# asonnino/hotstuff

Measured on NVIDIA H100. Metric: Ed25519 verifies/s, higher is better.
Workload: dtype u32

## Files before the change

hotstuff_b200/csrc/hs_engine.cu:

```cuda
#include <cuda_runtime.h>
#include <algorithm>
#include <array>
#include <atomic>
#include <condition_variable>
#include <cstdint>
#include <cstdio>
#include <cstdlib>
#include <cstring>
#include <deque>
#include <initializer_list>
#include <list>
#include <memory>
#include <mutex>
#include <new>
#include <optional>
#include <random>
#include <string>
#include <string_view>
#include <thread>
#include <unordered_map>
#include <vector>

#include "../../include/hs_crypto.h"
#include "hs_args.h"
#include "hs_selftest_vectors.h"
#include "verify_core.cuh"

#define HS_THREADS 128
#define HS_FINISH_GROUP 16
#define HS_NO_KEY 0xffffffffu
#define HS_LEARN_MAX 8192u
#define HS_LEARN_PER_CALL 1024u
#define HS_CACHE_RESET_MIN_CALLS 64u

struct in_layout {
  const uint8_t *sig;
  size_t sig_stride;
  const uint8_t *pk;
  size_t pk_stride;
  const uint32_t *vidx;
  const uint8_t *msg;
  size_t msg_stride;
  const uint32_t *midx;
  const uint64_t *off;
  uint64_t fixed_len;
  int aos128;
};

__device__ __forceinline__ void load32(uint32_t (&w)[8], const uint8_t *p) {
  const uint32_t *s = reinterpret_cast<const uint32_t *>(p);
#pragma unroll
  for (int i = 0; i < 8; i++) w[i] = __ldg(s + i);
}
__device__ __forceinline__ void unpack8(uint32_t (&w)[8], uint4 lo, uint4 hi) {
  w[0] = lo.x; w[1] = lo.y; w[2] = lo.z; w[3] = lo.w;
  w[4] = hi.x; w[5] = hi.y; w[6] = hi.z; w[7] = hi.w;
}
__device__ __forceinline__ void store_digest32(uint32_t *dst, const uint32_t *h) {
  uint4 *d = reinterpret_cast<uint4 *>(dst);
  d[0] = make_uint4(h[0], h[1], h[2], h[3]);
  d[1] = make_uint4(h[4], h[5], h[6], h[7]);
}
// ... 59 lines not shown
    h = (h + 1) & T.mask;
  }
  return HS_NO_KEY;
}
__global__ void __launch_bounds__(256) k_key_lookup(in_layout L, size_t n, key_table T, uint32_t *__restrict__ out_vidx,
                                                    uint32_t *__restrict__ miss_list, uint32_t *__restrict__ miss_count) {
  const size_t i = (size_t)blockIdx.x * 256 + threadIdx.x;
  if (i >= n) return;
  uint32_t k[8];
  load32(k, L.pk + i * L.pk_stride);
  uint32_t pos;
  const uint32_t found = key_probe<false>(T, k, pos);
  out_vidx[i] = found;
  if (found == HS_NO_KEY) miss_list[atomicAdd(miss_count, 1u)] = (uint32_t)i;
}

__global__ void __launch_bounds__(256) k_gather_keys(in_layout L, size_t n, const uint32_t *__restrict__ miss_list,
                                                     const uint32_t *__restrict__ miss_count, uint32_t max_keys, uint8_t *__restrict__ out_keys,
                                                     uint32_t *__restrict__ out_n) {
  const size_t t = (size_t)blockIdx.x * 256 + threadIdx.x;
  const size_t avail = miss_count ? (size_t)*miss_count : n;
  const size_t take = avail < max_keys ? avail : max_keys;
  if (t == 0) *out_n = (uint32_t)take;
  if (t >= take) return;
  const size_t i = miss_count ? miss_list[t] : t;
  uint32_t k[8];
  load32(k, L.pk + i * L.pk_stride);
  uint32_t *dst = reinterpret_cast<uint32_t *>(out_keys + t * 32);
#pragma unroll
  for (int j = 0; j < 8; j++) dst[j] = k[j];
}

struct main_out {
  fe *xyz;
  uint8_t *meta;
  int side_pass;
};
struct committee_tables {
  const uint8_t *pks;
  const uint8_t *key_flags;
  uint32_t n_keys;
  const ge_niels *atables;
  size_t table_entries;
};

template <bool COMMITTEE>
#ifndef HS_MAIN_MINBLOCKS
#define HS_MAIN_MINBLOCKS 4
#endif
#ifndef HS_GENERIC_MINBLOCKS
#define HS_GENERIC_MINBLOCKS 3
#endif
__global__ void __launch_bounds__(HS_THREADS, COMMITTEE ? HS_MAIN_MINBLOCKS : HS_GENERIC_MINBLOCKS) k_verify_main(in_layout L, size_t n_arg, const uint32_t *__restrict__ n_ptr,
                                                             const uint32_t *__restrict__ index_list, const ge_niels *__restrict__ btable,
                                                             committee_tables C, main_out O, const comb_params cp) {
  __shared__ __align__(16) unsigned char smem_raw[HS_MAX_DIGITS * HS_THREADS * 4];
  static_assert(sizeof(smem_raw) >= (HS_THREADS / 32) * 256 * sizeof(uint4), "staging does not fit");
  uint4(*stage)[256] = reinterpret_cast<uint4(*)[256]>(smem_raw);
  int32_t *digits = reinterpret_cast<int32_t *>(smem_raw) + threadIdx.x;
  const size_t n = n_ptr ? (size_t)*n_ptr : n_arg;
  for (size_t base = (size_t)blockIdx.x * blockDim.x; base < n; base += (size_t)gridDim.x * blockDim.x) {
  const size_t t = base + threadIdx.x;
  const size_t warp_first = t & ~(size_t)31;
  const bool active = t < n;
  size_t i = active ? t : n - 1;
  uint32_t R[8], S[8], A[8], h[16];
  uint32_t v = 0;
// ... 27 lines not shown
    if (len == 32 && ((reinterpret_cast<uintptr_t>(m) & 3u) == 0)) {
      uint32_t M[8];
      load32(M, m);
      sha512_ram32(h, R, A, M);
    } else {
      uint64_t pre[8];
#pragma unroll
      for (int j = 0; j < 4; j++) {
        pre[j] = be64_from_le32(R[2 * j], R[2 * j + 1]);
        pre[4 + j] = be64_from_le32(A[2 * j], A[2 * j + 1]);
      }
      sha512_prefix_msg(h, pre, 8, m, len);
    }
  }
  ge_ext acc;
  uint32_t meta;
  if (COMMITTEE) {
    meta = verify_committee_main(acc, R, S, h, btable, C.atables + (size_t)v * C.table_entries, have_key ? C.key_flags[v] : 0u, digits,
                                 HS_THREADS, cp);
    if (!have_key) {
      if (O.side_pass) continue;
      meta = 0;
    }
  } else {
    ge_cached tab[9];
    meta = verify_generic_main(acc, R, S, A, h, btable, tab, digits, HS_THREADS, cp);
  }
  if (!active) continue;
  if (!(meta & HS_META_PARSE_OK)) {
    fe_set0(acc.X);
    fe_set1(acc.Y);
    fe_set1(acc.Z);
  }
  uint4 *dst = reinterpret_cast<uint4 *>(O.xyz + i * 3);
  dst[0] = make_uint4(acc.X.v[0], acc.X.v[1], acc.X.v[2], acc.X.v[3]);
  dst[1] = make_uint4(acc.X.v[4], acc.X.v[5], acc.X.v[6], acc.X.v[7]);
  dst[2] = make_uint4(acc.Y.v[0], acc.Y.v[1], acc.Y.v[2], acc.Y.v[3]);
  dst[3] = make_uint4(acc.Y.v[4], acc.Y.v[5], acc.Y.v[6], acc.Y.v[7]);
  dst[4] = make_uint4(acc.Z.v[0], acc.Z.v[1], acc.Z.v[2], acc.Z.v[3]);
  dst[5] = make_uint4(acc.Z.v[4], acc.Z.v[5], acc.Z.v[6], acc.Z.v[7]);
  O.meta[i] = (uint8_t)meta;
  }
}

struct small_rec {
  uint8_t sig[64];
  uint8_t msg[32];
  uint32_t vidx;
  uint32_t req;
  uint32_t req_n;
  uint32_t pad[5];
};
static_assert(sizeof(small_rec) == 128, "small_rec is 128 bytes");
#define HS_SMALL_MAX 64
__device__ __forceinline__ void fe_shfl_down(fe &r, const fe &a, int delta) {
#pragma unroll
  for (int i = 0; i < 8; i++) r.v[i] = __shfl_down_sync(0xffffffffu, a.v[i], delta);
}

#define HS_SIG_WAYS 4
struct sig_entry {
  uint32_t w[32];
  uint32_t seq;
  uint32_t flags;
  uint32_t pad[2];
};
static_assert(sizeof(sig_entry) == 144, "sig_entry is 144 bytes");
struct sig_bucket {
  sig_entry e[HS_SIG_WAYS];
  uint32_t rr;
  uint32_t pad[3];
};
#define HS_SIG_CTRS 4
// ... 450 lines not shown
  int n;
  int my_rank;
  uint32_t epoch;
  size_t total_words;
  size_t word_offset;
};
#define HS_PEER_FLAGS(P) ((P).total_words * 2)
#define HS_PEER_CTRL(P) ((P).total_words * 2 + HS_MAX_PEERS)
__device__ __forceinline__ void peer_signal_and_wait(const peer_route &P) {
  const int p = threadIdx.x;
  if (p >= P.n) return;
  uint32_t *own = P.buf[P.my_rank];
  __threadfence_system();
  asm volatile("st.release.sys.global.u32 [%0], %1;" ::"l"(P.buf[p] + HS_PEER_FLAGS(P) + P.my_rank), "r"(P.epoch) : "memory");
  uint32_t v = 0;
  bool ok = false;
  for (long long spin = 0; spin < (1ll << 24); spin++) {
    asm volatile("ld.acquire.sys.global.u32 %0, [%1];" : "=r"(v) : "l"(own + HS_PEER_FLAGS(P) + p) : "memory");
    if ((int32_t)(v - P.epoch) >= 0) {
      ok = true;
      break;
    }
    __nanosleep(200);
  }
  if (!ok) {
    own[HS_PEER_CTRL(P)] = 1;
    const size_t per = P.total_words / P.n;
    uint32_t *w = own + (P.epoch & 1u) * P.total_words + (size_t)p * per;
    for (size_t k = 0; k < per; k++) w[k] = 0;
  }
}
__global__ void k_peer_sync_only(const peer_route P) { peer_signal_and_wait(P); }

__device__ __forceinline__ void fe_load_global(fe &r, const fe *p) {
  const uint4 *s = reinterpret_cast<const uint4 *>(p);
  unpack8(r.v, s[0], s[1]);
}
__host__ __device__ inline uint32_t mode_flag(uint32_t mode) { return mode == HS_MODE_BATCH_EQ ? HS_F_EQ : HS_F_STRICT; }
template <class Verdict>
__device__ __forceinline__ void verify_finish_body(const in_layout &L, size_t n, const fe *__restrict__ xyz, const uint8_t *__restrict__ meta,
                                                   Verdict verdict, uint32_t *__restrict__ bitmap, const peer_route &P, const int group) {
  __shared__ fe tot[HS_THREADS];
  const size_t t = (size_t)blockIdx.x * HS_THREADS + threadIdx.x;
  const size_t first = t * (size_t)group;
  const int cnt = (first < n) ? (int)((n - first < (size_t)group) ? (n - first) : group) : 0;
  fe prod[HS_FINISH_GROUP];
  fe run;
  fe_set1(run);
#pragma unroll 1
  for (int c = 0; c < cnt; c++) {
    fe Z;
    fe_load_global(Z, xyz + (first + c) * 3 + 2);
    if (fe_is_zero(Z)) fe_set1(Z);
    fe_mul(run, run, Z);
    prod[c] = run;
  }
  tot[threadIdx.x] = run;
  __syncthreads();
  block_invert4(tot);
  __syncthreads();
  uint32_t bits = 0;
  if (cnt) {
    fe u = tot[threadIdx.x];
#pragma unroll 1
    for (int c = cnt - 1; c >= 0; c--) {
      const size_t i = first + c;
      fe X, Y, Z, zinv;
      fe_load_global(X, xyz + i * 3 + 0);
      fe_load_global(Y, xyz + i * 3 + 1);
      fe_load_global(Z, xyz + i * 3 + 2);
      const uint32_t zero_z = fe_is_zero(Z);
      if (zero_z) fe_set1(Z);
      if (c > 0) fe_mul(zinv, u, prod[c - 1]);
      else zinv = u;
      fe_mul(u, u, Z);
      uint32_t R[8];
      load32(R, L.sig + i * L.sig_stride);
      uint32_t m = meta[i];
      if (zero_z) m &= ~HS_META_PARSE_OK;
      const uint32_t fl = verify_flags_from(X, Y, zinv, R, m);
      const uint32_t ok = verdict(i, fl);
      if (ok) bits |= 1u << c;
    }
  }
  const int lanes_per_word = 32 / group;
  uint32_t word = bits << (group * (threadIdx.x & (lanes_per_word - 1)));
  for (int m = 1; m < lanes_per_word; m <<= 1) word |= __shfl_xor_sync(0xffffffffu, word, m);
  if ((threadIdx.x & (lanes_per_word - 1)) == 0 && first < n) {
    const size_t widx = t / lanes_per_word;
    if (P.n == 0) {
      bitmap[widx] = word;
    } else {
      const size_t at = (P.epoch & 1u) * P.total_words + P.word_offset + widx;
#pragma unroll 1
      for (int p = 0; p < P.n; p++) P.buf[p][at] = word;
    }
  }
  if (P.n) {
    __shared__ int is_last;
    __threadfence_system();
    __syncthreads();
    if (threadIdx.x == 0) is_last = atomicAdd(P.buf[P.my_rank] + HS_PEER_CTRL(P) + 1, 1u) == gridDim.x - 1;
    __syncthreads();
    if (is_last) {
      peer_signal_and_wait(P);
      __syncthreads();
      if (threadIdx.x == 0) P.buf[P.my_rank][HS_PEER_CTRL(P) + 1] = 0;
    }
  }
}
__global__ void __launch_bounds__(HS_THREADS) k_verify_finish(in_layout L, size_t n, const fe *__restrict__ xyz, const uint8_t *__restrict__ meta,
                                                               uint32_t mode, uint32_t *__restrict__ bitmap, const peer_route P, const int group) {
  verify_finish_body(L, n, xyz, meta, [&](size_t, uint32_t fl) { return fl & mode_flag(mode); }, bitmap, P, group);
}
__global__ void __launch_bounds__(HS_THREADS) k_verify_finish_modes(in_layout L, size_t n, const fe *__restrict__ xyz, const uint8_t *__restrict__ meta,
                                                                     const uint8_t *__restrict__ item_mode, uint32_t *__restrict__ bitmap, const peer_route P,
                                                                     const int group) {
  verify_finish_body(L, n, xyz, meta, [&](size_t i, uint32_t fl) { return fl & mode_flag(item_mode[i]); }, bitmap, P, group);
}

#define HS_BUILD_BLOCK 64
__global__ void __launch_bounds__(HS_THREADS) k_build_comb(const uint8_t *__restrict__ encs, size_t n_points, int negate, int W, int n_windows,
                                                            ge_niels *tables, uint8_t *key_flags) {
  const int entries = 1 << (W - 1);
  const int blocks_per_window = entries / HS_BUILD_BLOCK;
  const size_t t = (size_t)blockIdx.x * HS_THREADS + threadIdx.x;
  const size_t per_point = (size_t)n_windows * blocks_per_window;
  const size_t p = t / per_point;
  if (p >= n_points) return;
  const int w = (int)((t % per_point) / blocks_per_window);
  const int b = (int)(t % blocks_per_window);
  ge_ext P;
  if (encs) {
    uint32_t e[8];
    load32(e, encs + p * 32);
    uint32_t ok = ge_decompress(P, e);
    uint32_t small = ge_enc_is_small_order(e);
    if (w == 0 && b == 0 && key_flags) key_flags[p] = (uint8_t)((ok & 1u) | (small << 1));
    if (!ok) ge_identity(P);
  } else {
    ge_basepoint(P);
  }
  if (negate) {
    ge_ext Q;
    ge_neg(Q, P);
    P = Q;
  }
  fe prod[HS_BUILD_BLOCK];
  comb_build_block(tables + p * ((size_t)n_windows * comb_window_stride(W)), P, W, w, b * HS_BUILD_BLOCK, HS_BUILD_BLOCK, prod);
}
// ... 643 lines not shown
  if (!c->cache_enabled || c->explicit_committee || c->learn_pending || !L.pk) return HS_OK;
  if (!c->learn.keys) {
    learn_bufs B;
    HS_CUDA(c, alloc(B.keys, (size_t)HS_LEARN_MAX * 32));
    HS_CUDA(c, alloc(B.n, 4));
    HS_CUDA(c, alloc(B.h_keys, (size_t)HS_LEARN_MAX * 32));
    HS_CUDA(c, alloc(B.h_n, 4));
    HS_CUDA(c, alloc(B.h_miss_total, 4));
    HS_CUDA(c, create(B.ev));
    HS_CUDA(c, create(B.ev_tables));
    c->learn = std::move(B);
  }
  learn_bufs &B = c->learn;
  c->learn_records = n;
  if (c->cache_full) {
    if (!have_lookup) return HS_OK;
    HS_CUDA(c, cudaMemcpyAsync(B.h_miss_total, c->d_miss_count, 4, cudaMemcpyDeviceToHost, stream));
    HS_CUDA(c, cudaEventRecord(B.ev, stream));
    c->learn_pending = true;
    return HS_OK;
  }
  k_gather_keys<<<blocks_for(HS_LEARN_MAX, 256), 256, 0, stream>>>(L, n, have_lookup ? (const uint32_t *)c->miss.p.get() : nullptr,
                                                                     have_lookup ? c->d_miss_count.get() : nullptr, HS_LEARN_MAX, B.keys, B.n);
  c->launches++;
  HS_CUDA(c, cudaGetLastError());
  HS_CUDA(c, cudaMemcpyAsync(B.h_n, B.n, 4, cudaMemcpyDeviceToHost, stream));
  HS_CUDA(c, cudaMemcpyAsync(B.h_keys, B.keys, (size_t)HS_LEARN_MAX * 32, cudaMemcpyDeviceToHost, stream));
  HS_CUDA(c, cudaEventRecord(B.ev, stream));
  c->learn_pending = true;
  return HS_OK;
}

struct pass_scratch {
  fe *xyz;
  uint8_t *meta;
  uint32_t *vidx, *miss, *miss_count;
  cudaStream_t side;
  cudaEvent_t ev_side[2];
  const event_h *prof;
};
struct pass_tables {
  committee_tables C;
  key_table T;
  comb_params cp;
};
static pass_tables ctx_tables(const hs_ctx *c) {
  return pass_tables{{c->keys.pks, c->keys.key_flags, (uint32_t)c->n_keys, c->keys.atables, c->a_table_entries},
                     {c->keys.slots, c->slot_mask, c->keys.pks, (uint32_t)c->n_keys}, c->cp};
}
template <class AfterLookup>
static int launch_main(hs_ctx *c, in_layout &L, size_t n, bool committee, bool indexed, const pass_tables &K, const pass_scratch &S,
                       cudaStream_t stream, AfterLookup after_lookup) {
  main_out O{S.xyz, S.meta, 0};
  const committee_tables &C = K.C;
  if (committee) {
    if (!indexed) {
      HS_CUDA(c, cudaMemsetAsync(S.miss_count, 0, 4, stream));
      k_key_lookup<<<blocks_for(n, 256), 256, 0, stream>>>(L, n, K.T, S.vidx, S.miss, S.miss_count);
      c->launches++;
      HS_CUDA(c, cudaGetLastError());
      L.vidx = S.vidx;
      O.side_pass = 1;
      HS_TRY(after_lookup(true));
      HS_CUDA(c, cudaEventRecord(S.ev_side[0], stream));
      HS_CUDA(c, cudaStreamWaitEvent(S.side, S.ev_side[0], 0));
      unsigned grid = blocks_for(n, 32);
      if (grid > c->n_sms * 8u) grid = c->n_sms * 8u;
      k_verify_main<false><<<grid, 32, 0, S.side>>>(L, 0, S.miss_count, S.miss, c->d_btable, C, O, K.cp);
      c->launches++;
      HS_CUDA(c, cudaGetLastError());
      HS_CUDA(c, cudaEventRecord(S.ev_side[1], S.side));
    }
    if (S.prof) HS_CUDA(c, cudaEventRecord(S.prof[0], stream));
    k_verify_main<true><<<blocks_for(n), HS_THREADS, 0, stream>>>(L, n, nullptr, nullptr, c->d_btable, C, O, K.cp);
    if (S.prof) HS_CUDA(c, cudaEventRecord(S.prof[1], stream));
    c->launches++;
    HS_CUDA(c, cudaGetLastError());
    if (!indexed) HS_CUDA(c, cudaStreamWaitEvent(stream, S.ev_side[1], 0));
  } else {
    HS_TRY(after_lookup(false));
    k_verify_main<false><<<blocks_for(n), HS_THREADS, 0, stream>>>(L, n, nullptr, nullptr, c->d_btable, C, O, K.cp);
    c->launches++;
    HS_CUDA(c, cudaGetLastError());
  }
  return HS_OK;
}
static int launch_finish(hs_ctx *c, const in_layout &L, size_t n, const fe *xyz, const uint8_t *meta, uint32_t mode, const uint8_t *d_item_mode,
                         uint32_t *d_bitmap, const peer_route &P, int fin_group, cudaStream_t stream) {
  const size_t fin_threads = (n + fin_group - 1) / fin_group;
  if (d_item_mode)
    k_verify_finish_modes<<<blocks_for(fin_threads), HS_THREADS, 0, stream>>>(L, n, xyz, meta, d_item_mode, d_bitmap, P, fin_group);
  else
    k_verify_finish<<<blocks_for(fin_threads), HS_THREADS, 0, stream>>>(L, n, xyz, meta, mode, d_bitmap, P, fin_group);
  c->launches++;
  HS_CUDA(c, cudaGetLastError());
  return HS_OK;
}

static int run_verify(hs_ctx *c, in_layout L, size_t n, uint32_t mode, uint32_t *d_bitmap, cudaStream_t stream, bool indexed,
                      const uint8_t *d_item_mode = nullptr) {
  if (n == 0) {
    if (c->peer_armed) {
      c->peer_armed = false;
      k_peer_sync_only<<<1, HS_MAX_PEERS, 0, stream>>>(c->peers);
      c->launches++;
      HS_CUDA(c, cudaGetLastError());
    }
    return HS_OK;
  }
  if (indexed && (!c->explicit_committee || c->n_keys == 0)) return fail(c, HS_ERR_ARG, "committee-indexed verify without a registered committee");
  if (!indexed) HS_TRY(learn_process(c, stream));
  if (c->learn.ev_tables && !c->explicit_committee) HS_CUDA(c, cudaStreamWaitEvent(stream, c->learn.ev_tables, 0));
  const bool defer = c->deferred && stream != c->stream;
  dev_buf &XYZ = (defer && c->flip) ? c->xyz2 : c->xyz, &META = (defer && c->flip) ? c->meta2 : c->meta;
  const int set = defer ? c->flip : 0;
  if (defer) {
    c->flip ^= 1;
    HS_CUDA(c, cudaStreamWaitEvent(stream, c->ev_tail[set], 0));
  }
  HS_TRY(ensure(c, XYZ, n * 3 * sizeof(fe)));
  HS_TRY(ensure(c, META, n));
  const bool committee = c->n_keys > 0 && (indexed || L.pk);
  if (!committee && !L.pk) return fail(c, HS_ERR_ARG, "verify without keys");
  if (committee && !indexed) {
    HS_TRY(ensure(c, c->vidx, n * 4));
    HS_TRY(ensure(c, c->miss, n * 4));
  }
  const pass_scratch S{(fe *)XYZ.p.get(), (uint8_t *)META.p.get(), (uint32_t *)c->vidx.p.get(), (uint32_t *)c->miss.p.get(), c->d_miss_count, c->stream_side,
                       {c->ev_side[0], c->ev_side[1]}, c->profile_main ? c->ev_prof : nullptr};
  HS_TRY(launch_main(c, L, n, committee, indexed, ctx_tables(c), S, stream,
                     [&](bool have_lookup) { return learn_collect(c, L, n, have_lookup, stream); }));
  const int fin_group = (defer || n >= (1u << 19)) ? 16 : (n >= (1u << 18) ? 8 : 4);
  peer_route P{};
  if (c->peer_armed) {
    P = c->peers;
    c->peer_armed = false;
  }
  cudaStream_t fin_stream = stream;
  if (defer) {
    HS_CUDA(c, cudaEventRecord(c->ev_main_done, stream));
    HS_CUDA(c, cudaStreamWaitEvent(c->stream_tail, c->ev_main_done, 0));
    fin_stream = c->stream_tail;
  }
  HS_TRY(launch_finish(c, L, n, (const fe *)XYZ.p.get(), (const uint8_t *)META.p.get(), mode, d_item_mode, d_bitmap, P, fin_group, fin_stream));
  if (defer) HS_CUDA(c, cudaEventRecord(c->ev_tail[set], c->stream_tail));
  return HS_OK;
}

static uint32_t host_key_lookup(const hs_ctx *c, const uint8_t *key) {
  if (c->n_keys == 0 || c->h_slots.empty()) return HS_NO_KEY;
  uint32_t w[8];
  memcpy(w, key, 32);
  uint32_t h = key_hash(w) & c->slot_mask;
  for (uint32_t probe = 0; probe <= c->slot_mask; probe++) {
    const uint32_t idx = c->h_slots[h];
    if (idx == HS_NO_KEY) return HS_NO_KEY;
    if (idx < c->n_keys && memcmp(c->h_pks.data() + 32 * (size_t)idx, key, 32) == 0) return idx;
    h = (h + 1) & c->slot_mask;
  }
  return HS_NO_KEY;
}
static bool small_eligible(const hs_ctx *c, size_t n) { return c->small_enabled && n >= 1 && n <= HS_SMALL_MAX && c->n_keys > 0 && c->keys.atables; }
struct small_src {
  const uint8_t *sig, *msg;
  uint32_t vidx;
};
template <class Rec>
static bool small_stage(hs_ctx *c, size_t n, Rec rec) {
  bool all = true;
  for (size_t i = 0; i < n; i++) {
    const small_src s = rec(i);
    memcpy(c->small.in.h[i].sig, s.sig, 64);
    memcpy(c->small.in.h[i].msg, s.msg, 32);
    c->small.in.h[i].vidx = s.vidx;
    all = all && s.vidx != HS_NO_KEY;
  }
  return all;
// ... 85 lines not shown
};
struct cert_span {
  std::string key;
  size_t h;
  std::vector<uint32_t> idx;
  uint8_t role;
};
enum { CERT_NEW, CERT_HIT, CERT_JOINED };
struct cert_req {
  ticket_sink sink;
  uint32_t n;
  std::vector<cert_span> spans;
  std::vector<uint32_t> ring_idx;
  uint32_t pending = 0;
  int status = HS_OK;
  std::vector<uint32_t> bits;
};
struct cert_flight {
  std::vector<std::pair<cert_req *, const cert_span *>> joiners;
};
struct generic_lists {
  mapped<uint32_t> slot;
  mapped<qmsg_desc> mlist;
};
struct sig_counters {
  dev_mem<uint64_t> key;
  dev_mem<uint32_t> ctr;
  mapped<uint32_t> hctr;
};
struct batch_lane {
  mapped<uint8_t> arena;
  dev_mem<uint8_t> mirror;
  dev_mem<uint32_t> dig;
  dev_mem<fe> xyz;
  dev_mem<uint8_t> meta;
  dev_mem<uint32_t> vidx, miss, miss_count, items, grej, counter;
  stream_h stream, side;
  event_h ev[2];
};
struct hs_queue {
  hs_ctx *c = nullptr;
  uint32_t cap = 0, mask = 0;
  mapped<small_rec> ring;
  mapped<uint8_t> flags;
  mapped<uint32_t> done;
  dev_mem<uint32_t> d_counters;
  mapped<uint8_t> pk;
  std::vector<uint8_t> modes;
  std::vector<uint32_t> wbits;
  stream_h stream;
  stream_h bulk_stream;
  event_h ev_last;
  event_h ev_bulk_last;
  uint64_t stats[HS_QUEUE_STATS] = {};
  byte_ring arena;
  mapped<uint8_t> arena_buf;
  dev_mem<uint8_t> d_stage;
  dev_mem<uint32_t> d_digs;
  mapped<qmsg_desc> mlist;
  uint64_t dstats[HS_QUEUE_DIGEST_STATS] = {};
  struct req {
    ticket_sink sink;
    uint32_t n;
    uint32_t seq;
    bool finished;
    bool msgs;
    uint32_t a_off, m, pre_bytes;
// ... 1333 lines not shown
  const size_t s_off = S.add(off, (n + 1) * 8), s_data = S.add(data, off[n], 8);
  HS_TRY(ensure(c, c->out, n * 32));
  HS_TRY(S.upload(c, c->in[0], c->stream));
  if (n <= 64 && off[n] / n >= 1024) {
    k_digest32_long<<<(unsigned)n, 32, 0, c->stream>>>(S.ptr(s_data), (const uint64_t *)S.ptr(s_off), n, (uint32_t *)c->out.p.get());
    c->launches++;
    HS_CUDA(c, cudaGetLastError());
  } else {
    HS_TRY(hs_digest32_dev(c, S.ptr(s_data), S.ptr(s_off), n, c->out.p, c->stream));
  }
  return readback(c, {{out, c->out.p.get(), n * 32}});
}

int hs_verify_msgs(hs_ctx *c, const uint8_t *sig, const uint8_t *pk, const uint32_t *vidx, const uint8_t *msgs, size_t msg_len, size_t n,
                   uint32_t mode, uint32_t *out_bitmap) {
  if (!c) return HS_ERR_ARG;
  if (const char *why = hs_args::msgs(sig, pk, vidx, msgs, msg_len, n, mode, out_bitmap)) return fail_args(c, "hs_verify_msgs", why);
  if (n == 0) return HS_OK;
  std::lock_guard<std::mutex> g(c->mu);
  HS_CUDA(c, cudaSetDevice(c->device));
  size_t CH = 1u << 17;
  if (const char *e = getenv("HS_CHUNK_RECORDS")) {
    size_t v = strtoull(e, nullptr, 10);
    if (v >= 1024) CH = v & ~(size_t)31;
  }
  const size_t key_bytes = vidx ? 4 : 32;
  const size_t per_rec = 64 + key_bytes + msg_len;
  const size_t chunk_cap = (n < CH ? n : CH);
  HS_TRY(ensure(c, c->out, ((n + 31) / 32) * 4));
  for (int b = 0; b < 2; b++) {
    HS_TRY(ensure(c, c->in[b], chunk_cap * per_rec + 64));
    HS_TRY(ensure(c, c->digest[b], chunk_cap * 32));
  }
  HS_TRY(ensure(c, c->xyz, chunk_cap * 3 * sizeof(fe)));
  HS_TRY(ensure(c, c->meta, chunk_cap));
  if (!vidx && c->n_keys) {
    HS_TRY(ensure(c, c->vidx, chunk_cap * 4));
    HS_TRY(ensure(c, c->miss, chunk_cap * 4));
  }
  size_t lo = 0;
  for (size_t j = 0; lo < n; j++) {
    const int b = (int)(j & 1);
    const size_t cnt = (n - lo < CH) ? (n - lo) : CH;
    uint8_t *d = (uint8_t *)c->in[b].p.get();
    const size_t o_sig = 0, o_key = cnt * 64, o_msg = o_key + ((cnt * key_bytes + 15) & ~(size_t)15);
    if (j >= 2) HS_CUDA(c, cudaStreamWaitEvent(c->stream2, c->ev_done[b], 0));
    HS_CUDA(c, cudaMemcpyAsync(d + o_sig, sig + lo * 64, cnt * 64, cudaMemcpyHostToDevice, c->stream2));
    if (vidx) HS_CUDA(c, cudaMemcpyAsync(d + o_key, vidx + lo, cnt * 4, cudaMemcpyHostToDevice, c->stream2));
    else HS_CUDA(c, cudaMemcpyAsync(d + o_key, pk + lo * 32, cnt * 32, cudaMemcpyHostToDevice, c->stream2));
    HS_CUDA(c, cudaMemcpyAsync(d + o_msg, msgs + lo * msg_len, cnt * msg_len, cudaMemcpyHostToDevice, c->stream2));
    HS_CUDA(c, cudaEventRecord(c->ev[b], c->stream2));
    HS_CUDA(c, cudaStreamWaitEvent(c->stream, c->ev[b], 0));
    HS_TRY(hs_verify_msgs_dev(c, d + o_sig, vidx ? nullptr : d + o_key, vidx ? d + o_key : nullptr, d + o_msg, msg_len, cnt, mode,
                              c->digest[b].p, (uint32_t *)c->out.p.get() + lo / 32, c->stream));
    HS_CUDA(c, cudaEventRecord(c->ev_done[b], c->stream));
    lo += cnt;
  }
  return readback(c, {{out_bitmap, c->out.p.get(), ((n + 31) / 32) * 4}});
}

int hs_queue_create(hs_ctx *c, size_t ring_records, hs_queue **out) {
  if (!c || !out || ring_records > HS_QUEUE_MAX_RECORDS) return fail(c, HS_ERR_ARG, "hs_queue_create: bad argument");
  *out = nullptr;
  uint32_t cap = HS_SMALL_MAX;
  while (cap < (ring_records ? ring_records : HS_QUEUE_DEFAULT_RECORDS)) cap <<= 1;
  HS_CUDA(c, cudaSetDevice(c->device));
  std::unique_ptr<hs_queue> q(new (std::nothrow) hs_queue());
// ... 385 lines not shown
  return queue_read_stats(q, "hs_queue_generic_stats", out, &hs_queue::gstats);
}

#define HS_QUEUE_BATCH_MAX_ITEMS (1u << 24)
#define HS_QUEUE_BATCH_MAX_BYTES (1ull << 30)
int hs_queue_batch(hs_queue *q, size_t max_items, size_t max_bytes) {
  if (!q || (max_items == 0) != (max_bytes == 0) || max_items > HS_QUEUE_BATCH_MAX_ITEMS || max_bytes > HS_QUEUE_BATCH_MAX_BYTES)
    return fail(q ? q->c : nullptr, HS_ERR_ARG, "hs_queue_batch: bad argument");
  hs_ctx *c = q->c;
  std::lock_guard<std::mutex> cfg(q->b_cfg_mu);
  {
    std::unique_lock<std::mutex> lk(q->mu);
    if (max_items == q->b_max_items && max_bytes == q->b_max_bytes) return HS_OK;
    q->b_max_items = q->b_max_bytes = 0;
    q->cv_done.wait(lk, [q] { return q->bq.empty(); });
  }
  HS_CUDA(c, cudaSetDevice(c->device));
  batch_drain(q);
  q->lane = {};
  q->b_arena = byte_ring{};
  if (!max_items) return HS_OK;
  uint64_t acap = 4096;
  while (acap < 2 * (uint64_t)max_bytes) acap <<= 1;
  batch_lane B;
  int lo = 0, hi = 0;
  cudaError_t e = cudaDeviceGetStreamPriorityRange(&lo, &hi);
  if (e == cudaSuccess) e = create(B.stream, lo);
  if (e == cudaSuccess) e = create(B.side, hi);
  for (event_h &ev : B.ev)
    if (e == cudaSuccess) e = create(ev);
  if (e == cudaSuccess) e = alloc(B.arena, acap);
  if (e == cudaSuccess) e = alloc(B.mirror, acap);
  if (e == cudaSuccess) e = alloc(B.dig, (max_bytes / 8 + 1) * 32);
  if (e == cudaSuccess) e = alloc(B.xyz, max_items * 3 * sizeof(fe));
  if (e == cudaSuccess) e = alloc(B.meta, max_items);
  if (e == cudaSuccess) e = alloc(B.vidx, max_items * 4);
  if (e == cudaSuccess) e = alloc(B.miss, max_items * 4);
  if (e == cudaSuccess) e = alloc(B.miss_count, 4);
  if (e == cudaSuccess) e = alloc(B.items, (max_items + 31) / 32 * 4);
  if (e == cudaSuccess) e = alloc(B.grej, max_bytes + 16);
  if (e == cudaSuccess) e = alloc(B.counter, 4);
  if (e == cudaSuccess) e = cudaMemset(B.counter, 0, 4);
  if (e != cudaSuccess) {
    cudaGetLastError();
    return fail(c, HS_ERR_NOMEM, "hs_queue_batch: no pinned host or device memory for the batch lane", e);
  }
  memset(B.arena.h, 0, acap);
  q->lane = std::move(B);
  std::lock_guard<std::mutex> g(q->mu);
  q->b_arena = byte_ring{acap, 0, 0};
  q->b_max_items = max_items;
  q->b_max_bytes = max_bytes;
  return HS_OK;
}

int hs_queue_submit_batch(hs_queue *q, const uint8_t *preimages, const uint64_t *pre_off, size_t n_msgs, const uint8_t *sig, const uint8_t *pk,
                          const uint32_t *msg_idx, const uint32_t *group_idx, const uint8_t *modes, size_t n_items, size_t n_groups, hs_queue_cb *cb,
                          void *user, size_t *out_ticket) {
  if (!q || !pre_off || !sig || !pk || !msg_idx || !group_idx || n_items == 0 || n_groups == 0 || n_msgs == 0 || n_items > HS_QUEUE_BATCH_MAX_ITEMS ||
      n_groups > UINT32_MAX || n_msgs > UINT32_MAX)
    return fail(q ? q->c : nullptr, HS_ERR_ARG, "hs_queue_submit_batch: bad argument");
  if (!offsets_ok(pre_off, n_msgs) || (pre_off[n_msgs] && !preimages)) return fail(q->c, HS_ERR_ARG, "hs_queue_submit_batch: bad preimage offsets");
  for (size_t i = 0; i < n_items; i++)
    if (msg_idx[i] >= n_msgs || group_idx[i] >= n_groups || (modes && modes[i] > HS_MODE_BATCH_EQ))
      return fail(q->c, HS_ERR_ARG, "hs_queue_submit_batch: index or mode out of range");
  const uint64_t pre_bytes = pre_off[n_msgs];
  const batch_layout B = batch_layout_of(n_msgs, pre_bytes, n_items, n_groups);
// ... 223 lines not shown
  if (e == cudaSuccess) e = alloc(KS.K.key_flags, n);
  if (e == cudaSuccess) e = alloc(KS.K.slots, (size_t)cap * 4);
  if (e == cudaSuccess) e = alloc(KS.K.atables, n * entries * sizeof(ge_niels));
  if (e != cudaSuccess) {
    cudaGetLastError();
    return fail(c, HS_ERR_NOMEM, "hs_self_test: the scratch key tables do not fit in device memory", e);
  }
  HS_CUDA(c, cudaMemcpyAsync(KS.K.pks, KS.pks.data(), n * 32, cudaMemcpyHostToDevice, st));
  HS_CUDA(c, cudaMemcpyAsync(KS.K.slots, KS.slots.data(), (size_t)cap * 4, cudaMemcpyHostToDevice, st));
  const size_t threads = n * (size_t)cp.na * ((1u << (cp.wa - 1)) / HS_BUILD_BLOCK);
  k_build_comb<<<blocks_for(threads), HS_THREADS, 0, st>>>(KS.K.pks, n, 1, cp.wa, cp.na, KS.K.atables, KS.K.key_flags);
  c->launches++;
  HS_CUDA(c, cudaGetLastError());
  K = pass_tables{{KS.K.pks, KS.K.key_flags, (uint32_t)n, KS.K.atables, entries}, {KS.K.slots, cap - 1, KS.K.pks, (uint32_t)n}, cp};
  return HS_OK;
}

static int st_verify_paths(hs_ctx *c, const st_set &T, const st_keys &KS, const pass_tables &K, cudaStream_t st, cudaStream_t side,
                           st_result &R) {
  const size_t n = T.r32.size(), nv = T.ev.size(), nmax = std::max(n, nv);
  std::vector<uint32_t> vidx(n);
  std::vector<uint8_t> modes(n);
  for (size_t i = 0; i < n; i++) {
    vidx[i] = KS.idx(T.r32[i].pk);
    modes[i] = (uint8_t)(i & 1);
  }
  const size_t words = (nmax + 31) / 32;
  dev_buf buf;
  h2d_stage S;
  const size_t s_recs = S.add(T.r32.data(), n * sizeof(hs_rec128)), s_vidx = S.add(vidx.data(), n * 4), s_modes = S.add(modes.data(), n),
               s_sig = S.add(T.sig.data(), nv * 64), s_pk = S.add(T.pk.data(), nv * 32), s_off = S.add(T.off.data(), (nv + 1) * 8),
               s_msg = S.add(T.msgs.data(), T.msgs.size(), 8);
  HS_TRY(S.upload(c, buf, st));
  dev_mem<fe> xyz;
  dev_mem<uint8_t> meta;
  dev_mem<uint32_t> lk, bm;
  HS_CUDA(c, alloc(xyz, nmax * 3 * sizeof(fe)));
  HS_CUDA(c, alloc(meta, nmax));
  HS_CUDA(c, alloc(lk, 2 * n * 4 + 4));
  HS_CUDA(c, alloc(bm, 3 * words * 4));
  event_h ev_side[2];
  for (event_h &ev : ev_side) HS_CUDA(c, create(ev));
  const st_drain drain{st, side};
  const pass_scratch PS{xyz, meta, lk, lk + n, lk + 2 * n, side, {ev_side[0], ev_side[1]}, nullptr};
  std::vector<uint32_t> strict(words), eq(words), mixed(words);
  auto pass = [&](uint32_t bit, const char *path, in_layout L, bool var, bool committee, bool indexed, uint32_t modes_bit) -> int {
    const size_t cnt = var ? nv : n;
    if (cnt == 0) return HS_OK;
    HS_CUDA(c, cudaMemsetAsync(bm, 0, 3 * words * 4, st));
    HS_TRY(launch_main(c, L, cnt, committee, indexed, K, PS, st, [](bool) { return HS_OK; }));
    HS_TRY(launch_finish(c, L, cnt, PS.xyz, PS.meta, HS_MODE_STRICT, nullptr, bm, peer_route{}, HS_SELFTEST_FIN_GROUP, st));
    HS_TRY(launch_finish(c, L, cnt, PS.xyz, PS.meta, HS_MODE_BATCH_EQ, nullptr, bm + words, peer_route{}, HS_SELFTEST_FIN_GROUP, st));
    if (modes_bit)
      HS_TRY(launch_finish(c, L, cnt, PS.xyz, PS.meta, HS_MODE_STRICT, S.ptr(s_modes), bm + 2 * words, peer_route{}, HS_SELFTEST_FIN_GROUP, st));
    HS_CUDA(c, cudaMemcpyAsync(strict.data(), bm, words * 4, cudaMemcpyDeviceToHost, st));
    HS_CUDA(c, cudaMemcpyAsync(eq.data(), bm + words, words * 4, cudaMemcpyDeviceToHost, st));
    HS_TRY(st_read(c, st, mixed.data(), bm + 2 * words, words * 4));
    st_compare(R, bit, path, var ? T.nv : T.n32, var ? T.ev : T.e32, nullptr, [&](size_t i) { return st_bitmap_bits(strict, eq, i); });
    if (modes_bit)
      st_compare(R, modes_bit, "k_verify_finish_modes", T.n32, T.e32, modes.data(),
                 [&](size_t i) { return (uint8_t)(((mixed[i >> 5] >> (i & 31)) & 1u) << modes[i]); });
    return HS_OK;
  };
  const uint8_t *recs = S.ptr(s_recs);
  HS_TRY(pass(HS_SELFTEST_GENERIC, "k_verify_main<generic> (packed records)", layout_rec128(recs), false, false, false, 0));
  HS_TRY(pass(HS_SELFTEST_VAR, "k_verify_main<generic> (variable-length messages)",
              in_layout{S.ptr(s_sig), 64, S.ptr(s_pk), 32, nullptr, S.ptr(s_msg), 0, nullptr, (const uint64_t *)S.ptr(s_off), 0, 0}, true, false, false, 0));
  HS_TRY(pass(HS_SELFTEST_COMMITTEE, "k_verify_main<committee> (committee indices)",
              in_layout{recs, 128, nullptr, 0, (const uint32_t *)S.ptr(s_vidx), recs + 96, 128, nullptr, nullptr, 32, 0}, false, true, true,
              HS_SELFTEST_MODES));
// ... 269 lines not shown
```

hotstuff_b200/csrc/verify_core.cuh:

```cuda
#pragma once
#include <cstdint>
#include "fe.cuh"
#include "ge.cuh"
#include "sc.cuh"
#include "sha512.cuh"

#define HS_F_PARSE_OK 1u
#define HS_F_EQ 4u
#define HS_F_SMALL 8u
#define HS_F_STRICT 16u

struct comb_params {
  int wa, na;
  int wb, nb;
  uint32_t bias_a[9], bias_b[9];
};
HS_HD size_t comb_window_stride(int w) { return ((size_t)1 << (w - 1)) + 1; }
HS_HD size_t comb_table_entries(int w) { return (size_t)sc_ndigits_rt(w) * comb_window_stride(w); }
#define HS_MAX_DIGITS 64

template <int W>
struct digits_msb {
  uint32_t u[8];
  HS_HD void init(const uint32_t (&s)[8]) {
// ... 202 lines not shown
#define HS_META_MISS 0x80u

HS_HD uint32_t verify_generic_main(ge_ext &acc, const uint32_t (&R)[8], const uint32_t (&S)[8], const uint32_t (&A)[8],
                                   const uint32_t (&h)[16], const ge_niels *btable, ge_cached *tab, int32_t *dig, int dig_stride,
                                   const comb_params &cp) {
  uint32_t k[8];
  sc_reduce512(k, h);
  uint32_t s_ok = sc_is_canonical(S);
  ge_ext Apt, negA;
  uint32_t a_ok = ge_decompress(Apt, A);
  uint32_t small = ge_enc_is_small_order(R) | ge_enc_is_small_order(A);
  ge_neg(negA, Apt);
  ge_scalarmult_window4(acc, negA, k, tab);
  sc_digits_rt(dig, dig_stride, S, cp.bias_b, cp.wb, cp.nb);
  ge_comb_accumulate_rt(acc, btable, dig, dig_stride, cp.wb, cp.nb);
  return ((s_ok & a_ok) ? HS_META_PARSE_OK : 0u) | (small ? HS_META_SMALL : 0u);
}
HS_HD uint32_t verify_committee_main(ge_ext &acc, const uint32_t (&R)[8], const uint32_t (&S)[8], const uint32_t (&h)[16],
                                     const ge_niels *btable, const ge_niels *neg_a_table, uint32_t a_flags, int32_t *dig, int dig_stride,
                                     const comb_params &cp) {
  uint32_t s_ok, small;
  {
    uint32_t k[8];
    sc_reduce512(k, h);
    s_ok = sc_is_canonical(S);
    small = ge_enc_is_small_order(R) | ((a_flags >> 1) & 1u);
    sc_digits_rt(dig, dig_stride, k, cp.bias_a, cp.wa, cp.na);
    sc_digits_rt(dig + cp.na * dig_stride, dig_stride, S, cp.bias_b, cp.wb, cp.nb);
  }
  ge_comb_ab(acc, neg_a_table, btable, dig, dig_stride, cp);
  return ((s_ok & a_flags & 1u) ? HS_META_PARSE_OK : 0u) | (small ? HS_META_SMALL : 0u);
}

HS_HD uint32_t verify_flags_from(const fe &X, const fe &Y, const fe &zinv, const uint32_t (&R)[8], uint32_t meta) {
  uint32_t parse_ok = meta & HS_META_PARSE_OK, small = (meta & HS_META_SMALL) ? 1u : 0u;
  uint32_t eq = (ge_matches_encoding(X, Y, zinv, R) && parse_ok) ? 1u : 0u;
  uint32_t fl = 0;
  if (parse_ok) fl |= HS_F_PARSE_OK;
  if (eq) fl |= HS_F_EQ;
  if (small) fl |= HS_F_SMALL;
  if (eq && !small) fl |= HS_F_STRICT;
  return fl;
}

HS_HD void comb_build_block(ge_niels *table, const ge_ext &P, int W, int win, int first, int count, fe *prod) {
  ge_ext base = P;
#if defined(__CUDA_ARCH__)
#pragma unroll 1
#endif
  for (int i = 0; i < W * win; i++) ge_dbl(base, base);
  ge_cached cb;
  ge_to_cached(cb, base);
  ge_ext m;
  ge_identity(m);
  const int mult = first + 1;
#if defined(__CUDA_ARCH__)
#pragma unroll 1
#endif
  for (int b = W; b >= 0; b--) {
    ge_dbl(m, m);
    if ((mult >> b) & 1) ge_add_cached(m, m, cb);
  }
  ge_niels *slot = table + (size_t)win * comb_window_stride(W) + 1 + first;
  if (first == 0) ge_niels_identity(slot[-1]);
  fe run;
  fe_set1(run);
// ... 201 lines not shown
```

Measured before the change: 258.0 million.

## Store projective results in warp-tiled SoA layout and interleave finish items per thread

```diff
diff --git a/hotstuff_b200/csrc/hs_engine.cu b/hotstuff_b200/csrc/hs_engine.cu
--- a/hotstuff_b200/csrc/hs_engine.cu
+++ b/hotstuff_b200/csrc/hs_engine.cu
@@ -27,7 +27,6 @@
 #include "verify_core.cuh"
 
 #define HS_THREADS 128
-#define HS_FINISH_GROUP 16
 #define HS_NO_KEY 0xffffffffu
 #define HS_LEARN_MAX 8192u
 #define HS_LEARN_PER_CALL 1024u
@@ -153,7 +152,7 @@
 }
 
 struct main_out {
-  fe *xyz;
+  uint32_t *xyz;
   uint8_t *meta;
   int side_pass;
 };
@@ -247,13 +246,7 @@
     fe_set1(acc.Y);
     fe_set1(acc.Z);
   }
-  uint4 *dst = reinterpret_cast<uint4 *>(O.xyz + i * 3);
-  dst[0] = make_uint4(acc.X.v[0], acc.X.v[1], acc.X.v[2], acc.X.v[3]);
-  dst[1] = make_uint4(acc.X.v[4], acc.X.v[5], acc.X.v[6], acc.X.v[7]);
-  dst[2] = make_uint4(acc.Y.v[0], acc.Y.v[1], acc.Y.v[2], acc.Y.v[3]);
-  dst[3] = make_uint4(acc.Y.v[4], acc.Y.v[5], acc.Y.v[6], acc.Y.v[7]);
-  dst[4] = make_uint4(acc.Z.v[0], acc.Z.v[1], acc.Z.v[2], acc.Z.v[3]);
-  dst[5] = make_uint4(acc.Z.v[4], acc.Z.v[5], acc.Z.v[6], acc.Z.v[7]);
+  xyz_store(O.xyz, i, acc.X, acc.Y, acc.Z);
   O.meta[i] = (uint8_t)meta;
   }
 }
@@ -770,68 +763,65 @@
 }
 __global__ void k_peer_sync_only(const peer_route P) { peer_signal_and_wait(P); }
 
-__device__ __forceinline__ void fe_load_global(fe &r, const fe *p) {
-  const uint4 *s = reinterpret_cast<const uint4 *>(p);
-  unpack8(r.v, s[0], s[1]);
-}
+#define HS_FIN_THREADS 128
+#define HS_FIN_MAX_GROUP 16
 __host__ __device__ inline uint32_t mode_flag(uint32_t mode) { return mode == HS_MODE_BATCH_EQ ? HS_F_EQ : HS_F_STRICT; }
 template <class Verdict>
-__device__ __forceinline__ void verify_finish_body(const in_layout &L, size_t n, const fe *__restrict__ xyz, const uint8_t *__restrict__ meta,
+__device__ __forceinline__ void verify_finish_body(const in_layout &L, size_t n, const uint32_t *__restrict__ xyz, const uint8_t *__restrict__ meta,
                                                    Verdict verdict, uint32_t *__restrict__ bitmap, const peer_route &P, const int group) {
-  __shared__ fe tot[HS_THREADS];
-  const size_t t = (size_t)blockIdx.x * HS_THREADS + threadIdx.x;
-  const size_t first = t * (size_t)group;
-  const int cnt = (first < n) ? (int)((n - first < (size_t)group) ? (n - first) : group) : 0;
-  fe prod[HS_FINISH_GROUP];
+  __shared__ fe tot[HS_FIN_THREADS];
+  const size_t base = (size_t)blockIdx.x * group * HS_FIN_THREADS + threadIdx.x;
+  fe prod[HS_FIN_MAX_GROUP];
   fe run;
   fe_set1(run);
 #pragma unroll 1
-  for (int c = 0; c < cnt; c++) {
-    fe Z;
-    fe_load_global(Z, xyz + (first + c) * 3 + 2);
-    if (fe_is_zero(Z)) fe_set1(Z);
-    fe_mul(run, run, Z);
-    prod[c] = run;
+  for (int j = 0; j < HS_FIN_MAX_GROUP; j++) {
+    const size_t i = base + (size_t)j * HS_FIN_THREADS;
+    if (j < group && i < n) {
+      fe Z;
+      xyz_load(Z, xyz, i, 2);
+      if (fe_is_zero(Z)) fe_set1(Z);
+      fe_mul(run, run, Z);
+    }
+    prod[j] = run;
   }
   tot[threadIdx.x] = run;
   __syncthreads();
   block_invert4(tot);
   __syncthreads();
-  uint32_t bits = 0;
-  if (cnt) {
-    fe u = tot[threadIdx.x];
+  fe u = tot[threadIdx.x];
+  const int lane = threadIdx.x & 31;
 #pragma unroll 1
-    for (int c = cnt - 1; c >= 0; c--) {
-      const size_t i = first + c;
+  for (int j = HS_FIN_MAX_GROUP - 1; j >= 0; j--) {
+    if (j >= group) continue;
+    const size_t i = base + (size_t)j * HS_FIN_THREADS;
+    uint32_t ok = 0;
+    if (i < n) {
       fe X, Y, Z, zinv;
-      fe_load_global(X, xyz + i * 3 + 0);
-      fe_load_global(Y, xyz + i * 3 + 1);
-      fe_load_global(Z, xyz + i * 3 + 2);
+      xyz_load(X, xyz, i, 0);
+      xyz_load(Y, xyz, i, 1);
+      xyz_load(Z, xyz, i, 2);
       const uint32_t zero_z = fe_is_zero(Z);
       if (zero_z) fe_set1(Z);
-      if (c > 0) fe_mul(zinv, u, prod[c - 1]);
+      if (j > 0) fe_mul(zinv, u, prod[j - 1]);
       else zinv = u;
       fe_mul(u, u, Z);
       uint32_t R[8];
       load32(R, L.sig + i * L.sig_stride);
       uint32_t m = meta[i];
       if (zero_z) m &= ~HS_META_PARSE_OK;
-      const uint32_t fl = verify_flags_from(X, Y, zinv, R, m);
-      const uint32_t ok = verdict(i, fl);
-      if (ok) bits |= 1u << c;
-    }
-  }
-  const int lanes_per_word = 32 / group;
-  uint32_t word = bits << (group * (threadIdx.x & (lanes_per_word - 1)));
-  for (int m = 1; m < lanes_per_word; m <<= 1) word |= __shfl_xor_sync(0xffffffffu, word, m);
-  if ((threadIdx.x & (lanes_per_word - 1)) == 0 && first < n) {
-    const size_t widx = t / lanes_per_word;
-    if (P.n == 0) {
-      bitmap[widx] = word;
-    } else {
-      const size_t at = (P.epoch & 1u) * P.total_words + P.word_offset + widx;
+      ok = verdict(i, verify_flags_from(X, Y, zinv, R, m)) ? 1u : 0u;
+    }
+    const uint32_t word = __ballot_sync(0xffffffffu, ok);
+    if (lane == 0 && i < n) {
+      const size_t widx = i >> 5;
+      if (P.n == 0) {
+        bitmap[widx] = word;
+      } else {
+        const size_t at = (P.epoch & 1u) * P.total_words + P.word_offset + widx;
 #pragma unroll 1
-      for (int p = 0; p < P.n; p++) P.buf[p][at] = word;
+        for (int p = 0; p < P.n; p++) P.buf[p][at] = word;
+      }
     }
   }
   if (P.n) {
@@ -847,13 +837,13 @@
     }
   }
 }
-__global__ void __launch_bounds__(HS_THREADS) k_verify_finish(in_layout L, size_t n, const fe *__restrict__ xyz, const uint8_t *__restrict__ meta,
-                                                               uint32_t mode, uint32_t *__restrict__ bitmap, const peer_route P, const int group) {
+__global__ void __launch_bounds__(HS_FIN_THREADS, 4) k_verify_finish(in_layout L, size_t n, const uint32_t *__restrict__ xyz, const uint8_t *__restrict__ meta,
+                                                                      uint32_t mode, uint32_t *__restrict__ bitmap, const peer_route P, const int group) {
   verify_finish_body(L, n, xyz, meta, [&](size_t, uint32_t fl) { return fl & mode_flag(mode); }, bitmap, P, group);
 }
-__global__ void __launch_bounds__(HS_THREADS) k_verify_finish_modes(in_layout L, size_t n, const fe *__restrict__ xyz, const uint8_t *__restrict__ meta,
-                                                                     const uint8_t *__restrict__ item_mode, uint32_t *__restrict__ bitmap, const peer_route P,
-                                                                     const int group) {
+__global__ void __launch_bounds__(HS_FIN_THREADS, 4) k_verify_finish_modes(in_layout L, size_t n, const uint32_t *__restrict__ xyz, const uint8_t *__restrict__ meta,
+                                                                            const uint8_t *__restrict__ item_mode, uint32_t *__restrict__ bitmap, const peer_route P,
+                                                                            const int group) {
   verify_finish_body(L, n, xyz, meta, [&](size_t i, uint32_t fl) { return fl & mode_flag(item_mode[i]); }, bitmap, P, group);
 }
 
@@ -1563,7 +1553,7 @@
 }
 
 struct pass_scratch {
-  fe *xyz;
+  uint32_t *xyz;
   uint8_t *meta;
   uint32_t *vidx, *miss, *miss_count;
   cudaStream_t side;
@@ -1595,9 +1585,9 @@
       HS_TRY(after_lookup(true));
       HS_CUDA(c, cudaEventRecord(S.ev_side[0], stream));
       HS_CUDA(c, cudaStreamWaitEvent(S.side, S.ev_side[0], 0));
-      unsigned grid = blocks_for(n, 32);
+      unsigned grid = blocks_for(n);
       if (grid > c->n_sms * 8u) grid = c->n_sms * 8u;
-      k_verify_main<false><<<grid, 32, 0, S.side>>>(L, 0, S.miss_count, S.miss, c->d_btable, C, O, K.cp);
+      k_verify_main<false><<<grid, HS_THREADS, 0, S.side>>>(L, 0, S.miss_count, S.miss, c->d_btable, C, O, K.cp);
       c->launches++;
       HS_CUDA(c, cudaGetLastError());
       HS_CUDA(c, cudaEventRecord(S.ev_side[1], S.side));
@@ -1616,13 +1606,13 @@
   }
   return HS_OK;
 }
-static int launch_finish(hs_ctx *c, const in_layout &L, size_t n, const fe *xyz, const uint8_t *meta, uint32_t mode, const uint8_t *d_item_mode,
+static int launch_finish(hs_ctx *c, const in_layout &L, size_t n, const uint32_t *xyz, const uint8_t *meta, uint32_t mode, const uint8_t *d_item_mode,
                          uint32_t *d_bitmap, const peer_route &P, int fin_group, cudaStream_t stream) {
-  const size_t fin_threads = (n + fin_group - 1) / fin_group;
+  const unsigned blocks = blocks_for((n + fin_group - 1) / fin_group, HS_FIN_THREADS);
   if (d_item_mode)
-    k_verify_finish_modes<<<blocks_for(fin_threads), HS_THREADS, 0, stream>>>(L, n, xyz, meta, d_item_mode, d_bitmap, P, fin_group);
+    k_verify_finish_modes<<<blocks, HS_FIN_THREADS, 0, stream>>>(L, n, xyz, meta, d_item_mode, d_bitmap, P, fin_group);
   else
-    k_verify_finish<<<blocks_for(fin_threads), HS_THREADS, 0, stream>>>(L, n, xyz, meta, mode, d_bitmap, P, fin_group);
+    k_verify_finish<<<blocks, HS_FIN_THREADS, 0, stream>>>(L, n, xyz, meta, mode, d_bitmap, P, fin_group);
   c->launches++;
   HS_CUDA(c, cudaGetLastError());
   return HS_OK;
@@ -1649,7 +1639,7 @@
     c->flip ^= 1;
     HS_CUDA(c, cudaStreamWaitEvent(stream, c->ev_tail[set], 0));
   }
-  HS_TRY(ensure(c, XYZ, n * 3 * sizeof(fe)));
+  HS_TRY(ensure(c, XYZ, xyz_bytes(n)));
   HS_TRY(ensure(c, META, n));
   const bool committee = c->n_keys > 0 && (indexed || L.pk);
   if (!committee && !L.pk) return fail(c, HS_ERR_ARG, "verify without keys");
@@ -1657,7 +1647,7 @@
     HS_TRY(ensure(c, c->vidx, n * 4));
     HS_TRY(ensure(c, c->miss, n * 4));
   }
-  const pass_scratch S{(fe *)XYZ.p.get(), (uint8_t *)META.p.get(), (uint32_t *)c->vidx.p.get(), (uint32_t *)c->miss.p.get(), c->d_miss_count, c->stream_side,
+  const pass_scratch S{(uint32_t *)XYZ.p.get(), (uint8_t *)META.p.get(), (uint32_t *)c->vidx.p.get(), (uint32_t *)c->miss.p.get(), c->d_miss_count, c->stream_side,
                        {c->ev_side[0], c->ev_side[1]}, c->profile_main ? c->ev_prof : nullptr};
   HS_TRY(launch_main(c, L, n, committee, indexed, ctx_tables(c), S, stream,
                      [&](bool have_lookup) { return learn_collect(c, L, n, have_lookup, stream); }));
@@ -1673,7 +1663,7 @@
     HS_CUDA(c, cudaStreamWaitEvent(c->stream_tail, c->ev_main_done, 0));
     fin_stream = c->stream_tail;
   }
-  HS_TRY(launch_finish(c, L, n, (const fe *)XYZ.p.get(), (const uint8_t *)META.p.get(), mode, d_item_mode, d_bitmap, P, fin_group, fin_stream));
+  HS_TRY(launch_finish(c, L, n, (const uint32_t *)XYZ.p.get(), (const uint8_t *)META.p.get(), mode, d_item_mode, d_bitmap, P, fin_group, fin_stream));
   if (defer) HS_CUDA(c, cudaEventRecord(c->ev_tail[set], c->stream_tail));
   return HS_OK;
 }
@@ -1825,7 +1815,7 @@
   mapped<uint8_t> arena;
   dev_mem<uint8_t> mirror;
   dev_mem<uint32_t> dig;
-  dev_mem<fe> xyz;
+  dev_mem<uint32_t> xyz;
   dev_mem<uint8_t> meta;
   dev_mem<uint32_t> vidx, miss, miss_count, items, grej, counter;
   stream_h stream, side;
@@ -3225,7 +3215,7 @@
     HS_TRY(ensure(c, c->in[b], chunk_cap * per_rec + 64));
     HS_TRY(ensure(c, c->digest[b], chunk_cap * 32));
   }
-  HS_TRY(ensure(c, c->xyz, chunk_cap * 3 * sizeof(fe)));
+  HS_TRY(ensure(c, c->xyz, xyz_bytes(chunk_cap)));
   HS_TRY(ensure(c, c->meta, chunk_cap));
   if (!vidx && c->n_keys) {
     HS_TRY(ensure(c, c->vidx, chunk_cap * 4));
@@ -3677,7 +3667,7 @@
   if (e == cudaSuccess) e = alloc(B.arena, acap);
   if (e == cudaSuccess) e = alloc(B.mirror, acap);
   if (e == cudaSuccess) e = alloc(B.dig, (max_bytes / 8 + 1) * 32);
-  if (e == cudaSuccess) e = alloc(B.xyz, max_items * 3 * sizeof(fe));
+  if (e == cudaSuccess) e = alloc(B.xyz, xyz_bytes(max_items));
   if (e == cudaSuccess) e = alloc(B.meta, max_items);
   if (e == cudaSuccess) e = alloc(B.vidx, max_items * 4);
   if (e == cudaSuccess) e = alloc(B.miss, max_items * 4);
@@ -3967,10 +3957,10 @@
                s_sig = S.add(T.sig.data(), nv * 64), s_pk = S.add(T.pk.data(), nv * 32), s_off = S.add(T.off.data(), (nv + 1) * 8),
                s_msg = S.add(T.msgs.data(), T.msgs.size(), 8);
   HS_TRY(S.upload(c, buf, st));
-  dev_mem<fe> xyz;
+  dev_mem<uint32_t> xyz;
   dev_mem<uint8_t> meta;
   dev_mem<uint32_t> lk, bm;
-  HS_CUDA(c, alloc(xyz, nmax * 3 * sizeof(fe)));
+  HS_CUDA(c, alloc(xyz, xyz_bytes(nmax)));
   HS_CUDA(c, alloc(meta, nmax));
   HS_CUDA(c, alloc(lk, 2 * n * 4 + 4));
   HS_CUDA(c, alloc(bm, 3 * words * 4));
diff --git a/hotstuff_b200/csrc/verify_core.cuh b/hotstuff_b200/csrc/verify_core.cuh
--- a/hotstuff_b200/csrc/verify_core.cuh
+++ b/hotstuff_b200/csrc/verify_core.cuh
@@ -258,6 +258,24 @@
   return ((s_ok & a_flags & 1u) ? HS_META_PARSE_OK : 0u) | (small ? HS_META_SMALL : 0u);
 }
 
+#define HS_XYZ_TILE_WORDS (3 * 8 * 32)
+HS_HD size_t xyz_bytes(size_t n) { return (n + 31) / 32 * HS_XYZ_TILE_WORDS * sizeof(uint32_t); }
+HS_HD size_t xyz_word(size_t i, int c) { return (i >> 5) * HS_XYZ_TILE_WORDS + (size_t)c * 256 + (i & 31); }
+HS_HD void xyz_store(uint32_t *xyz, size_t i, const fe &X, const fe &Y, const fe &Z) {
+  uint32_t *p = xyz + xyz_word(i, 0);
+#pragma unroll
+  for (int l = 0; l < 8; l++) {
+    p[l * 32] = X.v[l];
+    p[256 + l * 32] = Y.v[l];
+    p[512 + l * 32] = Z.v[l];
+  }
+}
+HS_HD void xyz_load(fe &r, const uint32_t *xyz, size_t i, int c) {
+  const uint32_t *p = xyz + xyz_word(i, c);
+#pragma unroll
+  for (int l = 0; l < 8; l++) r.v[l] = p[l * 32];
+}
+
 HS_HD uint32_t verify_flags_from(const fe &X, const fe &Y, const fe &zinv, const uint32_t (&R)[8], uint32_t meta) {
   uint32_t parse_ok = meta & HS_META_PARSE_OK, small = (meta & HS_META_SMALL) ? 1u : 0u;
   uint32_t eq = (ge_matches_encoding(X, Y, zinv, R) && parse_ok) ? 1u : 0u;
```

New measurement: 266.3 million, median of 6. +3.2%, better.
